# Zhen-Dong/CoDeNet

Measured on NVIDIA B200. Metric: CoDeNet1x 512x512 W4A8 forward + ctdet decode throughput, higher is better.
Workload: dtype int8

## Files before the change

### codenet_b200/csrc/decode.cu

```cuda
#include "layers.cuh"

#define DEC_THREADS 1024
#define DEC_BINS 2048
#define DEC_MAXK 1024

__device__ __forceinline__ uint32_t f2key(float f) {
  uint32_t b = __float_as_uint(f);
  return (b & 0x80000000u) ? ~b : (b | 0x80000000u);
}
__device__ __forceinline__ float key2f(uint32_t k) {
  uint32_t b = (k & 0x80000000u) ? (k & 0x7fffffffu) : ~k;
  return __uint_as_float(b);
}

struct DecParams {
  const float* hm; const float* wh; const float* reg;
  long long hm_is, wh_is, reg_is;
  int cat, H, W, K;
  int is_prob;
  unsigned long long* list;
  unsigned int* counts;
  float* dets; int32_t* inds;
};

__global__ void __launch_bounds__(256) ctdet_peaks_kernel(DecParams p, int batch) {
  const int HW = p.H * p.W;
  const unsigned n = (unsigned)p.cat * HW;
  const unsigned e = blockIdx.x * 256u + threadIdx.x;
  const int b = blockIdx.y, lane = threadIdx.x & 31;
  bool peak = false; float v = 0.f;
  if (e < n) {
    const int sp = (int)(e % (unsigned)HW); const int y = sp / p.W, x = sp - y * p.W;
    const float* plane = p.hm + (size_t)b * p.hm_is + (e - sp);
    v = __ldg(plane + sp);
    peak = (v == v);
#pragma unroll
    for (int dy = -1; dy <= 1; ++dy) {
      const int yy = y + dy; if ((unsigned)yy >= (unsigned)p.H) continue;
#pragma unroll
      for (int dx = -1; dx <= 1; ++dx) {
        const int xx = x + dx; if ((dx | dy) == 0 || (unsigned)xx >= (unsigned)p.W) continue;
        if (__ldg(plane + yy * p.W + xx) > v) peak = false;
      }
    }
  }
  __shared__ unsigned s_wcnt[8], s_base;
  const unsigned m = __ballot_sync(0xffffffffu, peak);
  const int warp = threadIdx.x >> 5;
  if (lane == 0) s_wcnt[warp] = __popc(m);
  __syncthreads();
  if (threadIdx.x == 0) {
    unsigned tot = 0;
#pragma unroll
    for (int w = 0; w < 8; ++w) { const unsigned c = s_wcnt[w]; s_wcnt[w] = tot; tot += c; }
    s_base = tot ? atomicAdd(p.counts + b, tot) : 0u;
  }
  __syncthreads();
  if (peak) p.list[(size_t)b * n + s_base + s_wcnt[warp] + __popc(m & ((1u << lane) - 1u))] =
      ((unsigned long long)f2key(v) << 32) | (unsigned long long)(0xffffffffu - e);
}

#define DEC_STRIP 16
__global__ void __launch_bounds__(256) ctdet_peaks_rows_kernel(DecParams p, int strips_per_plane) {
  pdl_launch_dependents();
  const int HW = p.H * p.W, W4 = p.W >> 2;
  const unsigned n = (unsigned)p.cat * HW;
  const int b = blockIdx.y, lane = threadIdx.x & 31, warp = threadIdx.x >> 5;
  const unsigned tid = blockIdx.x * 256u + threadIdx.x;
  const unsigned per_plane = (unsigned)strips_per_plane * W4;
  const unsigned plane_i = tid / per_plane, rem = tid - plane_i * per_plane;
  const bool live = plane_i < (unsigned)p.cat;
  const int strip = (int)(rem / W4), x0 = (int)(rem % W4) * 4;
  const float* plane = p.hm + (size_t)b * p.hm_is + (size_t)(live ? plane_i : 0) * HW;
  const int y0 = strip * DEC_STRIP, y1 = min(y0 + DEC_STRIP, p.H);
  const float NEG = -3.402823466e38f;
  auto load_row = [&](int y, float (&v)[4], float (&hm3)[4]) {
    if ((unsigned)y >= (unsigned)p.H || !live) { v[0] = v[1] = v[2] = v[3] = NEG; hm3[0] = hm3[1] = hm3[2] = hm3[3] = NEG; return; }
    const float* r = plane + (size_t)y * p.W + x0;
    const float4 q = __ldg((const float4*)r);
    const float l = x0 > 0 ? __ldg(r - 1) : NEG, rr = x0 + 4 < p.W ? __ldg(r + 4) : NEG;
    v[0] = q.x; v[1] = q.y; v[2] = q.z; v[3] = q.w;
    hm3[0] = fmaxf(fmaxf(l, q.x), q.y); hm3[1] = fmaxf(fmaxf(q.x, q.y), q.z);
    hm3[2] = fmaxf(fmaxf(q.y, q.z), q.w); hm3[3] = fmaxf(fmaxf(q.z, q.w), rr);
  };
  float vm[4], hmm[4], vc[4], hmc[4], vp[4], hmp[4];
  load_row(y0 - 1, vm, hmm); load_row(y0, vc, hmc);
  __shared__ unsigned s_wcnt[8], s_base;
  unsigned long long mask = 0ull;
  for (int y = y0; y < y1; ++y) {
    load_row(y + 1, vp, hmp);
#pragma unroll
    for (int i = 0; i < 4; ++i) {
      const float m = fmaxf(fmaxf(hmm[i], hmc[i]), hmp[i]);
      if (live && vc[i] == m) mask |= 1ull << ((y - y0) * 4 + i);
    }
#pragma unroll
    for (int i = 0; i < 4; ++i) { vm[i] = vc[i]; hmm[i] = hmc[i]; vc[i] = vp[i]; hmc[i] = hmp[i]; }
  }
  const unsigned cnt = (unsigned)__popcll(mask);
  unsigned incl = cnt;
#pragma unroll
  for (int o = 1; o < 32; o <<= 1) { const unsigned t = __shfl_up_sync(0xffffffffu, incl, o); if (lane >= o) incl += t; }
  if (lane == 31) s_wcnt[warp] = incl;
  __syncthreads();
  if (threadIdx.x == 0) {
    unsigned tot = 0;
#pragma unroll
    for (int w = 0; w < 8; ++w) { const unsigned c = s_wcnt[w]; s_wcnt[w] = tot; tot += c; }
    s_base = tot ? atomicAdd(p.counts + b, tot) : 0u;
  }
  __syncthreads();
  unsigned long long* dst = p.list + (size_t)b * n + s_base + s_wcnt[warp] + (incl - cnt);
  while (mask) {
    const int bit = __ffsll((long long)mask) - 1;
    mask &= mask - 1;
    const int y = y0 + (bit >> 2), x = x0 + (bit & 3);
    const float v = __ldg(plane + (size_t)y * p.W + x);
    const unsigned e = plane_i * HW + (unsigned)y * p.W + x;
    *dst++ = ((unsigned long long)f2key(v) << 32) | (unsigned long long)(0xffffffffu - e);
  }
}

__global__ void __launch_bounds__(DEC_THREADS) ctdet_decode_kernel(DecParams p) {
  __shared__ unsigned int hist[DEC_BINS];
  __shared__ unsigned long long sel[DEC_MAXK];
  __shared__ unsigned int s_count, s_nsel;
  __shared__ unsigned long long s_prefix, s_mask;
  __shared__ unsigned int s_krem, s_done;
  __shared__ unsigned int warp_sums[32];

  const int b = blockIdx.x, tid = threadIdx.x, lane = tid & 31, warp = tid >> 5;
  const int HW = p.H * p.W;
  const long long n = (long long)p.cat * HW;
  const float* hm = p.hm + (size_t)b * p.hm_is;
  unsigned long long* list = p.list + (size_t)b * n;

  if (tid == 0) { s_count = p.counts[b]; s_nsel = 0; }
  __syncthreads();
  const unsigned int count = s_count;
  const unsigned int Ksel = min((unsigned)p.K, count);

  if (tid == 0) { s_prefix = 0ull; s_mask = 0ull; s_krem = Ksel; s_done = (Ksel == 0 || Ksel == count) ? 1u : 0u; }
  __syncthreads();
  for (int shift = 53; !s_done; shift = max(shift - 11, 0)) {
    const int width = (shift == 0) ? 9 : 11;
    const unsigned nb = 1u << width;
    for (int i = tid; i < DEC_BINS; i += DEC_THREADS) hist[i] = 0;
    __syncthreads();
    const unsigned long long prefix = s_prefix, mask = s_mask;
    for (unsigned i = tid; i < count; i += DEC_THREADS) {
      unsigned long long c = list[i];
      if ((c & mask) == prefix) atomicAdd(&hist[(unsigned)(c >> shift) & (nb - 1)], 1u);
    }
    __syncthreads();
    {
      unsigned d0 = nb - 1 - 2 * tid, d1 = nb - 2 - 2 * tid;
      unsigned c0 = (2 * tid < nb) ? hist[d0] : 0u, c1 = (2 * tid + 1 < nb) ? hist[d1] : 0u;
      unsigned mine = c0 + c1, incl = mine;
      for (int o = 1; o < 32; o <<= 1) { unsigned t = __shfl_up_sync(0xffffffffu, incl, o); if (lane >= o) incl += t; }
      if (lane == 31) warp_sums[warp] = incl;
      __syncthreads();
      unsigned woff = 0;
      for (int w2 = 0; w2 < warp; ++w2) woff += warp_sums[w2];
      unsigned before = woff + incl - mine;
      const unsigned krem = s_krem;
      __syncthreads();
      if (2 * tid < nb && before < krem && krem <= before + c0) {
        s_prefix = prefix | ((unsigned long long)d0 << shift);
        s_mask = mask | ((unsigned long long)(nb - 1) << shift);
        s_krem = krem - before;
        if (krem == before + c0 || shift == 0) s_done = 1u;
      } else if (2 * tid + 1 < nb && before + c0 < krem && krem <= before + c0 + c1) {
        s_prefix = prefix | ((unsigned long long)d1 << shift);
        s_mask = mask | ((unsigned long long)(nb - 1) << shift);
        s_krem = krem - before - c0;
        if (krem == before + c0 + c1 || shift == 0) s_done = 1u;
      }
      __syncthreads();
    }
    if (shift == 0) break;
  }
  __syncthreads();
  const unsigned long long thr = (Ksel == count) ? 0ull : s_prefix;
  for (unsigned i = tid; i < count && Ksel > 0; i += DEC_THREADS) {
    unsigned long long c = list[i];
    if (c >= thr) { unsigned pos = atomicAdd(&s_nsel, 1u); if (pos < DEC_MAXK) sel[pos] = c; }
  }
  __syncthreads();
  unsigned nsel = min(s_nsel, (unsigned)DEC_MAXK);
  unsigned np2 = 1; while (np2 < nsel) np2 <<= 1;
  for (unsigned i = nsel + tid; i < np2; i += DEC_THREADS) sel[i] = 0ull;
  __syncthreads();
  for (unsigned k2 = 2; k2 <= np2; k2 <<= 1)
    for (unsigned j = k2 >> 1; j > 0; j >>= 1) {
      for (unsigned i = tid; i < np2; i += DEC_THREADS) {
        unsigned ixj = i ^ j;
        if (ixj > i) {
          unsigned long long a = sel[i], c = sel[ixj];
          bool desc = ((i & k2) == 0);
          if (desc ? (a < c) : (a > c)) { sel[i] = c; sel[ixj] = a; }
        }
      }
      __syncthreads();
    }
  for (int i = tid; i < p.K; i += DEC_THREADS) {
    float* d = p.dets + ((size_t)b * p.K + i) * 6;
    if ((unsigned)i < nsel && (unsigned)i < Ksel) {
      unsigned long long c = sel[i];
      uint32_t flat = 0xffffffffu - (uint32_t)(c & 0xffffffffull);
      float logit = key2f((uint32_t)(c >> 32));
      int cls = flat / HW, sp = flat - cls * HW;
      float xs = (float)(sp % p.W), ys = (float)(sp / p.W);
      if (p.reg) { xs += p.reg[(size_t)b * p.reg_is + sp]; ys += p.reg[(size_t)b * p.reg_is + HW + sp]; }
      else { xs += 0.5f; ys += 0.5f; }
      float w = p.wh[(size_t)b * p.wh_is + sp], h = p.wh[(size_t)b * p.wh_is + HW + sp];
      d[0] = xs - w / 2; d[1] = ys - h / 2; d[2] = xs + w / 2; d[3] = ys + h / 2;
      d[4] = p.is_prob ? logit : (float)(1.0 / (1.0 + exp(-(double)logit)));
      d[5] = (float)cls;
      if (p.inds) p.inds[(size_t)b * p.K + i] = (int32_t)flat;
    } else {
      d[0] = d[1] = d[2] = d[3] = d[4] = d[5] = 0.f;
      if (p.inds) p.inds[(size_t)b * p.K + i] = -1;
    }
  }
}

int decode_launch(const float* hm, long long hm_img_stride, const float* wh, long long wh_img_stride, const float* reg,
                  long long reg_img_stride, int batch, int cat, int H, int W, int K, int is_prob,
                  unsigned long long* scratch, unsigned int* counts, float* dets, int32_t* inds, cudaStream_t st) {
  CDN_CHECK(K >= 1 && K <= DEC_MAXK, CDN_ERR_INVALID, "decode: K=%d must be in 1..%d", K, DEC_MAXK);
  CDN_CHECK(cat >= 1 && H >= 1 && W >= 1 && (long long)cat * H * W < (1ll << 31), CDN_ERR_INVALID, "decode: bad shape");
  CDN_CHECK(hm && wh && dets && scratch && counts, CDN_ERR_INVALID, "decode: null pointer");
  CDN_CHECK(batch <= 65535, CDN_ERR_INVALID, "decode: batch %d exceeds 65535", batch);
  if (batch == 0) return 0;
  DecParams p{hm, wh, reg, hm_img_stride, wh_img_stride, reg_img_stride, cat, H, W, K, is_prob, scratch, counts, dets, inds};
  CDN_CUDA(cudaMemsetAsync(counts, 0, (size_t)batch * sizeof(unsigned int), st));
  const unsigned n = (unsigned)cat * H * W;
  if (W % 4 == 0 && (((uintptr_t)hm | (uintptr_t)(hm_img_stride * 4)) & 15) == 0) {
    const int strips = (H + DEC_STRIP - 1) / DEC_STRIP;
    const unsigned threads = (unsigned)cat * strips * (W / 4);
    ctdet_peaks_rows_kernel<<<dim3((threads + 255) / 256, batch), 256, 0, st>>>(p, strips);
    CDN_LAUNCH_CHECK("ctdet_peaks_rows_kernel");
  } else {
    ctdet_peaks_kernel<<<dim3((n + 255) / 256, batch), 256, 0, st>>>(p, batch);
    CDN_LAUNCH_CHECK("ctdet_peaks_kernel");
  }
  ctdet_decode_kernel<<<batch, DEC_THREADS, 0, st>>>(p);
  CDN_LAUNCH_CHECK("ctdet_decode_kernel");
  return 0;
}

__global__ void ctdet_post_affine_kernel(float* dets, const double* trans, int K, long long total) {
  const long long i = (long long)blockIdx.x * blockDim.x + threadIdx.x;
  if (i >= total) return;
  const double* t = trans + (i / K) * 6;
  float* d = dets + i * 6;
#pragma unroll
  for (int c = 0; c < 2; ++c) {
    const double x = (double)d[2 * c], y = (double)d[2 * c + 1];
    const double nx = __dadd_rn(__dadd_rn(__dmul_rn(t[0], x), __dmul_rn(t[1], y)), t[2]);
    const double ny = __dadd_rn(__dadd_rn(__dmul_rn(t[3], x), __dmul_rn(t[4], y)), t[5]);
    d[2 * c] = (float)nx; d[2 * c + 1] = (float)ny;
  }
}

extern "C" int cdn_ctdet_post_affine(float* d_dets, int batch, int K, const double* h_trans, cdn_stream_t stream) {
  CDN_CHECK(d_dets && h_trans && batch >= 0 && K >= 1, CDN_ERR_INVALID, "post_affine: bad arguments");
  if (batch == 0) return 0;
  double* d_t = nullptr;
  CDN_CUDA(cudaMalloc(&d_t, (size_t)batch * 6 * sizeof(double)));
// ... 40 lines not shown
```

### codenet_b200/csrc/engine.cu

```cuda
#include "layers.cuh"
#include <algorithm>
#include <mutex>

static thread_local char g_err[1024] = "";
unsigned g_cdn_debug_flags = 0;

int cdn_fail(int code, const char* fmt, ...) {
  va_list ap; va_start(ap, fmt); vsnprintf(g_err, sizeof(g_err), fmt, ap); va_end(ap);
  return code;
}
std::mutex& cdn_attr_mutex() { static std::mutex m; return m; }
int cdn_num_sms() {
  static int sms[64] = {};
  int dev = 0;
  if (cudaGetDevice(&dev) != cudaSuccess || dev < 0 || dev >= 64) return 148;
  std::lock_guard<std::mutex> lk(cdn_attr_mutex());
  if (!sms[dev]) { cudaDeviceGetAttribute(&sms[dev], cudaDevAttrMultiProcessorCount, dev); if (sms[dev] <= 0) sms[dev] = 148; }
  return sms[dev];
}

int dev_requant_upload(DevRequant& d, const cdn_requant* rq, const int32_t* acc_bias_host, int n_pad) {
  CDN_CHECK(rq && rq->n <= n_pad, CDN_ERR_INVALID, "requant: n=%d exceeds padded size %d", rq ? rq->n : -1, n_pad);
  std::vector<float> Mh(n_pad, 0.f), Bh(n_pad, 0.f), thr(n_pad, 0.5f);
  std::vector<double> M(n_pad, 0.0), B(n_pad, 0.0);
// ... 225 lines not shown
  if (int r = dw_device_build(L->dw, wq, sc->ws, C, pitch, zx, rq)) { delete L; return r; }
  if (int r = deform_scale_build(L->dw, &L->sc, L->ws.data(), C, zx)) { dw_device_free(L->dw); delete L; return r; }
  *out = L;
  return 0;
}
extern "C" int cdn_deform_layer_run(cdn_deform_layer* L, const int8_t* d_in, int in_pitch, int batch, int H, int W, int in_shift,
                                    int8_t* d_out, int out_pitch, float* d_sval, cdn_stream_t stream) {
  CDN_CHECK(L != nullptr, CDN_ERR_INVALID, "null deform layer");
  CDN_CHECK(std::min(in_pitch, out_pitch) >= L->Cp, CDN_ERR_INVALID, "deform layer: pitch smaller than the layer's %d", L->Cp);
  return deform_launch(L->dw, &L->sc, d_in, in_pitch, d_out, out_pitch, batch, H, W, in_shift, L->zx, d_sval, (cudaStream_t)stream);
}
extern "C" int cdn_deform_layer_destroy(cdn_deform_layer* L) {
  if (!L) return 0;
  cudaSetDevice(L->device);
  dw_device_free(L->dw);
  delete L;
  return 0;
}

static int decode_standalone(const float* d_hm, const float* d_wh, const float* d_reg, int batch, int cat, int H, int W,
                             int K, int is_prob, float* d_dets, int32_t* d_inds, cdn_stream_t stream) {
  unsigned long long* scratch = nullptr;
  CDN_CHECK(batch >= 0 && cat >= 1 && H >= 1 && W >= 1, CDN_ERR_INVALID, "decode: bad shape");
  size_t n = (size_t)batch * cat * H * W;
  CDN_CUDA(cudaMalloc(&scratch, (n ? n : 1) * sizeof(unsigned long long) + ((size_t)batch + 1) * sizeof(unsigned int)));
  long long hw = (long long)H * W;
  int r = decode_launch(d_hm, cat * hw, d_wh, 2 * hw, d_reg, 2 * hw, batch, cat, H, W, K, is_prob, scratch,
                        (unsigned int*)(scratch + (n ? n : 1)), d_dets, d_inds, (cudaStream_t)stream);
  cudaError_t e = cudaStreamSynchronize((cudaStream_t)stream);
  if (!r && e != cudaSuccess) r = cdn_fail(CDN_ERR_CUDA, "decode: %s", cudaGetErrorString(e));
  cudaFree(scratch);
  return r;
}
extern "C" size_t cdn_ctdet_decode_ws_bytes(int batch, int cat, int H, int W) {
  if (batch < 0 || cat < 1 || H < 1 || W < 1) return 0;
  size_t n = (size_t)batch * cat * H * W;
  return (n ? n : 1) * sizeof(unsigned long long) + ((size_t)batch + 1) * sizeof(unsigned int);
}
extern "C" int cdn_ctdet_decode_ws(const float* d_hm, long long hm_img_stride, const float* d_wh, long long wh_img_stride,
                                   const float* d_reg, long long reg_img_stride, int batch, int cat, int H, int W,
                                   int K, int is_prob, float* d_dets, int32_t* d_inds, void* d_ws, size_t ws_bytes,
                                   cdn_stream_t stream) {
  CDN_CHECK(batch >= 0 && cat >= 1 && H >= 1 && W >= 1, CDN_ERR_INVALID, "decode: bad shape");
  CDN_CHECK(d_ws && ((uintptr_t)d_ws & 7) == 0 && ws_bytes >= cdn_ctdet_decode_ws_bytes(batch, cat, H, W), CDN_ERR_INVALID,
            "decode: workspace of %zu bytes (8-byte aligned) needed, got %zu", cdn_ctdet_decode_ws_bytes(batch, cat, H, W), ws_bytes);
  size_t n = (size_t)batch * cat * H * W;
  long long hw = (long long)H * W;
  CDN_CHECK((!hm_img_stride || hm_img_stride >= cat * hw) && (!wh_img_stride || wh_img_stride >= 2 * hw) &&
            (!reg_img_stride || reg_img_stride >= 2 * hw), CDN_ERR_INVALID, "decode: image stride smaller than one image");
  unsigned long long* scratch = (unsigned long long*)d_ws;
  return decode_launch(d_hm, hm_img_stride ? hm_img_stride : cat * hw, d_wh, wh_img_stride ? wh_img_stride : 2 * hw, d_reg,
                       reg_img_stride ? reg_img_stride : 2 * hw, batch, cat, H, W, K, is_prob, scratch,
                       (unsigned int*)(scratch + (n ? n : 1)), d_dets, d_inds, (cudaStream_t)stream);
}
extern "C" int cdn_ctdet_decode(const float* d_hm, const float* d_wh, const float* d_reg, int batch, int cat, int H, int W,
                                int K, float* d_dets, int32_t* d_inds, cdn_stream_t stream) {
  return decode_standalone(d_hm, d_wh, d_reg, batch, cat, H, W, K, 0, d_dets, d_inds, stream);
}
extern "C" int cdn_ctdet_decode_prob(const float* d_heat, const float* d_wh, const float* d_reg, int batch, int cat, int H,
                                     int W, int K, float* d_dets, int32_t* d_inds, cdn_stream_t stream) {
  return decode_standalone(d_heat, d_wh, d_reg, batch, cat, H, W, K, 1, d_dets, d_inds, stream);
}

struct EngTensor { int H, W, pitch; int8_t* ptr; };
struct EngOp {
  int kind;
  int in_t, pass_t, out_t, in_shift, stride, pool, zx, H, W;
  StemDevice stem; DwDevice dw; PwDevice pw; cdn_deform_scale sc; std::vector<int8_t> ws_host;
  CUtensorMap tmA, tmP, tmO;
};

struct cdn_engine {
  int device = 0, max_batch = 0, finalized = 0;
  int in_H = 0, in_W = 0;
  std::vector<EngTensor> tensors;
  std::vector<EngOp*> ops;
// ... 162 lines not shown
}

extern "C" int cdn_engine_set_heads(cdn_engine* e, int cat, int H, int W, int K, int has_reg) {
  ENG_CHECK(e);
  CDN_CHECK(cat > 0 && H > 0 && W > 0 && K > 0 && K <= 1024, CDN_ERR_INVALID, "heads: bad arguments");
  e->cat = cat; e->hH = H; e->hW = W; e->K = K; e->has_reg = has_reg;
  return 0;
}

extern "C" int cdn_engine_finalize(cdn_engine* e, int max_batch) {
  ENG_CHECK(e);
  CDN_CHECK(!e->finalized, CDN_ERR_STATE, "engine already finalized");
  CDN_CHECK(max_batch > 0 && !e->ops.empty() && e->cat > 0, CDN_ERR_INVALID, "finalize: empty plan, heads not set, or bad batch");
  CDN_CHECK(e->n_f32 == e->cat + 2 + (e->has_reg ? 2 : 0), CDN_ERR_INVALID, "finalize: head conv has %d fp32 planes, expected %d", e->n_f32, e->cat + 2 + (e->has_reg ? 2 : 0));
  CDN_CUDA(cudaSetDevice(e->device));
  e->max_batch = max_batch;
  for (auto& t : e->tensors) {
    size_t bytes = (size_t)max_batch * t.H * t.W * t.pitch;
    CDN_CUDA(cudaMalloc((void**)&t.ptr, bytes));
    CDN_CUDA(cudaMemset(t.ptr, 0, bytes));
  }
  size_t ppi = (size_t)e->hH * e->hW;
  CDN_CUDA(cudaMalloc((void**)&e->heads, (size_t)max_batch * e->n_f32 * ppi * sizeof(float)));
  CDN_CUDA(cudaMalloc((void**)&e->dec_scratch, (size_t)max_batch * e->cat * ppi * sizeof(unsigned long long) + ((size_t)max_batch + 1) * sizeof(unsigned int)));
  CDN_CUDA(cudaMalloc((void**)&e->dets, (size_t)max_batch * e->K * 6 * sizeof(float)));
  CDN_CUDA(cudaMalloc((void**)&e->inds, (size_t)max_batch * e->K * sizeof(int32_t)));
  for (auto* op : e->ops) {
    if (op->kind == 0 && op->pool) {
      size_t b = (size_t)max_batch * ((op->H - 1) / op->stride + 1) * ((op->W - 1) / op->stride + 1) * 32;
      CDN_CUDA(cudaMalloc((void**)&e->stem_tmp, b));
    }
    if (op->kind == 3) {
      const EngTensor& ti = e->tensors[op->in_t];
      uint64_t rows = (uint64_t)max_batch * ti.H * ti.W;
      if (int r = make_tmap_2d(&op->tmA, ti.ptr, ti.pitch, rows, ti.pitch, 128)) return r;
      if (op->pass_t >= 0) { const EngTensor& tp = e->tensors[op->pass_t]; if (int r = make_tmap_2d(&op->tmP, tp.ptr, tp.pitch, rows, tp.pitch, 128)) return r; }
      if (op->out_t >= 0) { const EngTensor& to = e->tensors[op->out_t]; if (int r = make_tmap_2d(&op->tmO, to.ptr, to.pitch, rows, to.pitch, 128)) return r; }
    }
  }
  CDN_CUDA(cudaDeviceSynchronize());
  e->finalized = 1;
  return 0;
}

static bool engine_fuses_heads(const cdn_engine* e, size_t oi) {
  if (!e->fuse_heads || (g_cdn_debug_flags & 256u) || oi + 1 >= e->ops.size()) return false;
  const EngOp *a = e->ops[oi], *b = e->ops[oi + 1];
// ... 95 lines not shown
        int out_pitch = op->out_t >= 0 ? e->tensors[op->out_t].pitch : 0;
        r = pw_launch(op->pw, ti.ptr, ti.pitch, (long long)batch * ti.H * ti.W, pass, pass_pitch, out, out_pitch,
                      op->out_t < 0 ? e->heads : nullptr, e->hH * e->hW, &op->tmA, op->pass_t >= 0 ? &op->tmP : nullptr,
                      op->out_t >= 0 ? &op->tmO : nullptr, st);
        launches++;
      } break;
    }
    if (r) return r;
    mark();
  }
  const long long ppi = (long long)e->hH * e->hW;
  if (d_hm || d_wh || d_reg) {
    long long total = (long long)batch * e->n_f32 * ppi;
    heads_copyout_kernel<<<(unsigned)((total + 255) / 256), 256, 0, st>>>(e->heads, e->n_f32, e->cat, (int)ppi, total, d_hm, d_wh, d_reg, e->hm_logits);
    CDN_LAUNCH_CHECK("heads_copyout_kernel");
    launches++;
  }
  mark();
  if (d_dets) {
    const float* hm = e->heads;
    const float* wh = e->heads + (size_t)e->cat * ppi;
    const float* reg = e->has_reg ? e->heads + (size_t)(e->cat + 2) * ppi : nullptr;
    long long is = (long long)e->n_f32 * ppi;
    if (int r = decode_launch(hm, is, wh, is, reg, is, batch, e->cat, e->hH, e->hW, e->K, 0, e->dec_scratch,
                              (unsigned int*)(e->dec_scratch + (size_t)e->max_batch * e->cat * ppi), d_dets, d_inds, st)) return r;
    launches += 2;
  }
  mark();
  e->launches = launches;
  return 0;
}

extern "C" int cdn_engine_profile(cdn_engine* e, const float* d_img, int batch, float* ms, int n, cdn_stream_t stream) {
  ENG_CHECK(e);
  CDN_CHECK(e->finalized && batch > 0 && batch <= e->max_batch && d_img && ms, CDN_ERR_INVALID, "profile: bad arguments");
  CDN_CHECK(n >= (int)e->ops.size() + 2, CDN_ERR_INVALID, "profile: need room for %d timings", (int)e->ops.size() + 2);
  CDN_CUDA(cudaSetDevice(e->device));
  std::vector<cudaEvent_t> marks;
  int r = engine_enqueue(e, d_img, 0, batch, nullptr, nullptr, nullptr, e->dets, e->inds, (cudaStream_t)stream, &marks);
  cudaError_t ce = cudaStreamSynchronize((cudaStream_t)stream);
  if (!r && ce != cudaSuccess) r = cdn_fail(CDN_ERR_CUDA, "profile: %s", cudaGetErrorString(ce));
  for (int i = 0; i < n; ++i) ms[i] = 0.f;
  if (!r) for (size_t i = 0; i + 1 < marks.size() && (int)i < n; ++i) cudaEventElapsedTime(&ms[i], marks[i], marks[i + 1]);
  for (auto ev : marks) cudaEventDestroy(ev);
  return r;
}

static int engine_run_any(cdn_engine* e, const void* d_img, int is_u8, int batch, float* d_hm, float* d_wh, float* d_reg,
// ... 200 lines not shown
```

### codenet_b200/csrc/layers.cuh

```cuda
#pragma once
#include "common.cuh"

struct DwDevice {
  uint32_t *wA = nullptr, *wB = nullptr, *wC = nullptr, *ws = nullptr;
  uint32_t *wpk1 = nullptr, *wpk2 = nullptr, *wpku = nullptr;
  float2* mb = nullptr; int32_t* abm = nullptr; float thr = 0.5f, thr_bil = 0.01f; int u_ok = 1;
  RqInt* ki = nullptr; int use_int = 0;
  int sh0 = 0;
  uint32_t* pad_px = nullptr;
  int32_t* s_thr = nullptr; int s_n = 0, s_lo = 0, s_mode0_ok = 0;
  DevRequant rq;
  int cw_total = 0;
  long long acc_s_bias = 0;
};
int dw_device_build(DwDevice& d, const int8_t* wq, const int8_t* ws, int C, int Cp, int zx, const cdn_requant* rq);
int deform_scale_build(DwDevice& d, const cdn_deform_scale* sc, const int8_t* ws, int C, int zx);
void dw_device_free(DwDevice& d);
int dw_launch(const DwDevice& d, const int8_t* in, int in_pitch, int8_t* out, int out_pitch, int batch, int H, int W,
              int in_shift, int stride, int zx, cudaStream_t st);
bool dw_tma_ok(const DwDevice& d, int in_pitch, int out_pitch, int H, int W, int in_shift, int stride);
int dw_tma_launch(const DwDevice& d, const int8_t* in, int in_pitch, int8_t* out, int out_pitch, int batch, int H, int W,
                  int stride, int zx, cudaStream_t st);
int deform_launch(const DwDevice& d, const cdn_deform_scale* sc, const int8_t* in, int in_pitch, int8_t* out,
                  int out_pitch, int batch, int H, int W, int in_shift, int zx, float* sval, cudaStream_t st);
// ... 36 lines not shown
int pw_launch(const PwDevice& d, const int8_t* in, int in_pitch, long long pixels, const int8_t* pass, int pass_pitch,
              int8_t* out, int out_pitch, float* out_f32, int ppi, const CUtensorMap* tmA, const CUtensorMap* tmP,
              const CUtensorMap* tmO, cudaStream_t st);
bool heads_fused_ok(const DwDevice& dw, const PwDevice& pw, int in_pitch, int mid_pitch, int Hs, int Ws);
int heads_fused_launch(const DwDevice& dw, const PwDevice& pw, const int8_t* in, int in_pitch, int batch, int Hs, int Ws,
                       int zx, float* out_f32, cudaStream_t st);
bool unit_fused_ok(const PwDevice& pw1, const DwDevice& dw, const PwDevice& pw3, int x_pitch, int mid_pitch, int out_pitch, int H, int W);
int unit_fused_launch(const PwDevice& pw1, const DwDevice& dw, const PwDevice& pw3, const int8_t* x, int8_t* out, int HP,
                      int batch, int H, int W, int zx_mid, int8_t* dump_c1, int8_t* dump_d2, cudaStream_t st);
bool unit_fused_ws_ok(const PwDevice& pw1, const DwDevice& dw, const PwDevice& pw3, int x_pitch, int mid_pitch, int out_pitch, int H, int W);
int unit_fused_ws_launch(const PwDevice& pw1, const DwDevice& dw, const PwDevice& pw3, const int8_t* x, int8_t* out,
                         int batch, int H, int W, int zx_mid, int8_t* dump_c1, int8_t* dump_d2, cudaStream_t st);
int make_tmap_nhwc_swz(CUtensorMap* m, const void* base, uint64_t pitch, uint64_t W, uint64_t H, uint64_t batch,
                       uint32_t box_c, uint32_t box_w, uint32_t box_h);
bool unit_s2_fused_ok(const PwDevice& pw1, const DwDevice& dw, const PwDevice& pw3, int x_pitch, int mid_pitch, int pass_pitch,
                      int out_pitch, int H, int W);
int unit_s2_fused_launch(const PwDevice& pw1, const DwDevice& dw, const PwDevice& pw3, const int8_t* x, const int8_t* pass, int pass_pitch,
                         int8_t* out, int batch, int H, int W, int zx_mid, int8_t* dump_c1, int8_t* dump_d2, cudaStream_t st);
int make_tmap_nhwc(CUtensorMap* m, const void* base, uint64_t pitch, uint64_t W, uint64_t H, uint64_t batch, uint32_t box_w, uint32_t box_h);
int make_tmap_2d(CUtensorMap* m, const void* base, uint64_t cols, uint64_t rows, uint64_t pitch, uint32_t box_rows);

int decode_launch(const float* hm, long long hm_img_stride, const float* wh, long long wh_img_stride, const float* reg,
                  long long reg_img_stride, int batch, int cat, int H, int W, int K, int is_prob,
                  unsigned long long* scratch, unsigned int* counts, float* dets, int32_t* inds, cudaStream_t st);
```

Measured before the change: 93520.

## Replace global peak list with per-block local top-K slots before final selection

Each peak-finding block now keeps a shared histogram of its local peaks and runs a radix top-K select, writing at most K candidates into a fixed per-block slot region. The old design appended every peak to one global list through an atomic counter. The final decode kernel then runs radix select over the much smaller slot array, staging it in dynamic shared memory when it fits, and the counts memset is removed. This cuts global traffic and the cost of the single-block selection, but adds per-block selection work and zero-padded slots.

New measurement: 93270, median of 6. No clear change (-0.3%).

```diff
diff --git a/codenet_b200/csrc/decode.cu b/codenet_b200/csrc/decode.cu
--- a/codenet_b200/csrc/decode.cu
+++ b/codenet_b200/csrc/decode.cu
@@ -1,8 +1,17 @@
 #include "layers.cuh"
 
+#include <algorithm>
+
+#ifndef DEC_THREADS
 #define DEC_THREADS 1024
+#endif
+#define DEC_RT 256
+#define DEC_STRIP 16
+#define DEC_EPT 16
 #define DEC_BINS 2048
 #define DEC_MAXK 1024
+#define DEC_STAGE 2048
+#define DEC_SMEM_CAND 12288
 
 __device__ __forceinline__ uint32_t f2key(float f) {
   uint32_t b = __float_as_uint(f);
@@ -11,6 +20,9 @@
 __device__ __forceinline__ float key2f(uint32_t k) {
   uint32_t b = (k & 0x80000000u) ? (k & 0x7fffffffu) : ~k;
   return __uint_as_float(b);
+}
+__device__ __forceinline__ unsigned long long composite(float v, unsigned e) {
+  return ((unsigned long long)f2key(v) << 32) | (unsigned long long)(0xffffffffu - e);
 }
 
 struct DecParams {
@@ -18,22 +30,114 @@
   long long hm_is, wh_is, reg_is;
   int cat, H, W, K;
   int is_prob;
-  unsigned long long* list;
-  unsigned int* counts;
+  int rpp, spr, kslot;
+  unsigned nslots;
+  unsigned long long* slots;
   float* dets; int32_t* inds;
 };
 
-__global__ void __launch_bounds__(256) ctdet_peaks_kernel(DecParams p, int batch) {
+struct DecSel { unsigned warp[32]; unsigned res[4]; unsigned pos, nst; };
+
+template <int NT>
+__device__ void radix_find(const unsigned* hist, unsigned nb, unsigned krem, DecSel& s) {
+  const unsigned t = threadIdx.x, lane = t & 31, warp = t >> 5;
+  const unsigned per = (nb + NT - 1) / NT, r0 = t * per;
+  unsigned mine = 0;
+  for (unsigned j = 0; j < per && r0 + j < nb; ++j) mine += hist[nb - 1 - r0 - j];
+  unsigned incl = mine;
+#pragma unroll
+  for (int o = 1; o < 32; o <<= 1) { const unsigned v = __shfl_up_sync(0xffffffffu, incl, o); if (lane >= (unsigned)o) incl += v; }
+  if (lane == 31) s.warp[warp] = incl;
+  __syncthreads();
+  unsigned before = incl - mine, total = 0;
+#pragma unroll
+  for (unsigned w = 0; w < NT / 32; ++w) { const unsigned c = s.warp[w]; total += c; if (w < warp) before += c; }
+  if (before < krem && krem <= before + mine) {
+    for (unsigned j = 0;; ++j) {
+      const unsigned d = nb - 1 - r0 - j, c = hist[d];
+      if (krem <= before + c) { s.res[0] = d; s.res[1] = before; s.res[2] = c; break; }
+      before += c;
+    }
+  }
+  if (t == 0) s.res[3] = total;
+  __syncthreads();
+}
+
+template <int NT, class Each>
+__device__ unsigned long long topk_threshold(Each&& each, unsigned* hist, unsigned kk, DecSel& s, unsigned& total) {
+  __syncthreads();
+  unsigned nb = DEC_BINS, krem = kk;
+  int shift = 53;
+  radix_find<NT>(hist, nb, krem, s);
+  total = s.res[3];
+  if (total <= kk) return 0ull;
+  unsigned long long prefix = 0ull, pmask = 0ull;
+  for (;;) {
+    prefix |= (unsigned long long)s.res[0] << shift;
+    pmask |= (unsigned long long)(nb - 1) << shift;
+    krem -= s.res[1];
+    if (krem == s.res[2] || shift == 0) return prefix;
+    shift = max(shift - 11, 0);
+    nb = shift ? DEC_BINS : 512;
+    for (unsigned i = threadIdx.x; i < nb; i += NT) hist[i] = 0;
+    __syncthreads();
+    each([&](unsigned long long c) {
+      if ((c & pmask) == prefix) atomicAdd(&hist[(unsigned)(c >> shift) & (nb - 1)], 1u);
+    });
+    __syncthreads();
+    radix_find<NT>(hist, nb, krem, s);
+  }
+}
+
+template <class Each>
+__device__ void region_topk(Each&& each, unsigned* hist, DecSel& s, unsigned kslot, unsigned long long* out) {
+  __shared__ unsigned long long stage[DEC_STAGE];
+  if (threadIdx.x == 0) { s.pos = 0; s.nst = 0; }
+  __syncthreads();
+  radix_find<DEC_RT>(hist, DEC_BINS, kslot, s);
+  const unsigned total = s.res[3], d1 = s.res[0], c1 = s.res[2];
+  if (total <= kslot) {
+    each([&](unsigned long long c) { out[atomicAdd(&s.pos, 1u)] = c; });
+    for (unsigned i = total + threadIdx.x; i < kslot; i += DEC_RT) out[i] = 0ull;
+    return;
+  }
+  if (c1 <= DEC_STAGE) {
+    const unsigned krem = kslot - s.res[1];
+    each([&](unsigned long long c) {
+      const unsigned d = (unsigned)(c >> 53);
+      if (d > d1) out[atomicAdd(&s.pos, 1u)] = c;
+      else if (d == d1) stage[atomicAdd(&s.nst, 1u)] = c;
+    });
+    for (unsigned i = threadIdx.x; i < DEC_BINS; i += DEC_RT) hist[i] = 0;
+    __syncthreads();
+    if (threadIdx.x == 0) hist[d1] = c1;
+    auto each_staged = [&](auto&& f) { for (unsigned i = threadIdx.x; i < c1; i += DEC_RT) f(stage[i]); };
+    unsigned t;
+    const unsigned long long thr = topk_threshold<DEC_RT>(each_staged, hist, krem, s, t);
+    each_staged([&](unsigned long long c) { if (c >= thr) out[atomicAdd(&s.pos, 1u)] = c; });
+    return;
+  }
+  unsigned t;
+  const unsigned long long thr = topk_threshold<DEC_RT>(each, hist, kslot, s, t);
+  each([&](unsigned long long c) { if (c >= thr) out[atomicAdd(&s.pos, 1u)] = c; });
+}
+
+__global__ void __launch_bounds__(DEC_RT) ctdet_peaks_kernel(DecParams p) {
+  __shared__ unsigned s_hist[DEC_BINS];
+  __shared__ DecSel s;
+  for (unsigned i = threadIdx.x; i < DEC_BINS; i += DEC_RT) s_hist[i] = 0;
   const int HW = p.H * p.W;
-  const unsigned n = (unsigned)p.cat * HW;
-  const unsigned e = blockIdx.x * 256u + threadIdx.x;
-  const int b = blockIdx.y, lane = threadIdx.x & 31;
-  bool peak = false; float v = 0.f;
-  if (e < n) {
-    const int sp = (int)(e % (unsigned)HW); const int y = sp / p.W, x = sp - y * p.W;
-    const float* plane = p.hm + (size_t)b * p.hm_is + (e - sp);
-    v = __ldg(plane + sp);
-    peak = (v == v);
+  const int b = blockIdx.y, plane_i = blockIdx.x / p.rpp, sp0 = (blockIdx.x - plane_i * p.rpp) * (DEC_RT * DEC_EPT);
+  const float* plane = p.hm + (size_t)b * p.hm_is + (size_t)plane_i * HW;
+  __syncthreads();
+  unsigned mask = 0;
+#pragma unroll 4
+  for (int j = 0; j < DEC_EPT; ++j) {
+    const int sp = sp0 + j * DEC_RT + threadIdx.x;
+    if (sp >= HW) break;
+    const int y = sp / p.W, x = sp - y * p.W;
+    const float v = __ldg(plane + sp);
+    bool peak = (v == v) && (v >= -3.402823466e38f || (y > 0 && y < p.H - 1 && x > 0 && x < p.W - 1));
 #pragma unroll
     for (int dy = -1; dy <= 1; ++dy) {
       const int yy = y + dy; if ((unsigned)yy >= (unsigned)p.H) continue;
@@ -43,153 +147,116 @@
         if (__ldg(plane + yy * p.W + xx) > v) peak = false;
       }
     }
-  }
-  __shared__ unsigned s_wcnt[8], s_base;
-  const unsigned m = __ballot_sync(0xffffffffu, peak);
-  const int warp = threadIdx.x >> 5;
-  if (lane == 0) s_wcnt[warp] = __popc(m);
-  __syncthreads();
-  if (threadIdx.x == 0) {
-    unsigned tot = 0;
-#pragma unroll
-    for (int w = 0; w < 8; ++w) { const unsigned c = s_wcnt[w]; s_wcnt[w] = tot; tot += c; }
-    s_base = tot ? atomicAdd(p.counts + b, tot) : 0u;
-  }
-  __syncthreads();
-  if (peak) p.list[(size_t)b * n + s_base + s_wcnt[warp] + __popc(m & ((1u << lane) - 1u))] =
-      ((unsigned long long)f2key(v) << 32) | (unsigned long long)(0xffffffffu - e);
-}
-
-#define DEC_STRIP 16
-__global__ void __launch_bounds__(256) ctdet_peaks_rows_kernel(DecParams p, int strips_per_plane) {
+    if (peak) { mask |= 1u << j; atomicAdd(&s_hist[f2key(v) >> 21], 1u); }
+  }
+  const unsigned base = (unsigned)plane_i * HW;
+  region_topk([&](auto&& f) {
+    for (unsigned m = mask; m; m &= m - 1) {
+      const int sp = sp0 + (__ffs(m) - 1) * DEC_RT + threadIdx.x;
+      f(composite(__ldg(plane + sp), base + sp));
+    }
+  }, s_hist, s, p.kslot, p.slots + ((size_t)b * gridDim.x + blockIdx.x) * p.kslot);
+}
+
+__global__ void __launch_bounds__(DEC_RT) ctdet_peaks_rows_kernel(DecParams p) {
   pdl_launch_dependents();
+  __shared__ unsigned s_hist[DEC_BINS];
+  __shared__ DecSel s;
+  for (unsigned i = threadIdx.x; i < DEC_BINS; i += DEC_RT) s_hist[i] = 0;
   const int HW = p.H * p.W, W4 = p.W >> 2;
-  const unsigned n = (unsigned)p.cat * HW;
-  const int b = blockIdx.y, lane = threadIdx.x & 31, warp = threadIdx.x >> 5;
-  const unsigned tid = blockIdx.x * 256u + threadIdx.x;
-  const unsigned per_plane = (unsigned)strips_per_plane * W4;
-  const unsigned plane_i = tid / per_plane, rem = tid - plane_i * per_plane;
-  const bool live = plane_i < (unsigned)p.cat;
-  const int strip = (int)(rem / W4), x0 = (int)(rem % W4) * 4;
-  const float* plane = p.hm + (size_t)b * p.hm_is + (size_t)(live ? plane_i : 0) * HW;
-  const int y0 = strip * DEC_STRIP, y1 = min(y0 + DEC_STRIP, p.H);
+  const int b = blockIdx.y, plane_i = blockIdx.x / p.rpp, r = blockIdx.x - plane_i * p.rpp;
+  const int ls = threadIdx.x / W4, x0 = (threadIdx.x - ls * W4) * 4;
+  const int y0 = (r * p.spr + ls) * DEC_STRIP, y1 = min(y0 + DEC_STRIP, p.H);
+  const float* plane = p.hm + (size_t)b * p.hm_is + (size_t)plane_i * HW;
   const float NEG = -3.402823466e38f;
-  auto load_row = [&](int y, float (&v)[4], float (&hm3)[4]) {
-    if ((unsigned)y >= (unsigned)p.H || !live) { v[0] = v[1] = v[2] = v[3] = NEG; hm3[0] = hm3[1] = hm3[2] = hm3[3] = NEG; return; }
-    const float* r = plane + (size_t)y * p.W + x0;
-    const float4 q = __ldg((const float4*)r);
-    const float l = x0 > 0 ? __ldg(r - 1) : NEG, rr = x0 + 4 < p.W ? __ldg(r + 4) : NEG;
-    v[0] = q.x; v[1] = q.y; v[2] = q.z; v[3] = q.w;
-    hm3[0] = fmaxf(fmaxf(l, q.x), q.y); hm3[1] = fmaxf(fmaxf(q.x, q.y), q.z);
-    hm3[2] = fmaxf(fmaxf(q.y, q.z), q.w); hm3[3] = fmaxf(fmaxf(q.z, q.w), rr);
+  struct Row { float4 q; float l, r; };
+  auto load_row = [&](int y) {
+    Row o;
+    if ((unsigned)y < (unsigned)p.H) {
+      const float* rp = plane + (size_t)y * p.W + x0;
+      o.q = __ldg((const float4*)rp);
+      o.l = x0 > 0 ? __ldg(rp - 1) : NEG; o.r = x0 + 4 < p.W ? __ldg(rp + 4) : NEG;
+    } else {
+      o.q = make_float4(NEG, NEG, NEG, NEG); o.l = o.r = NEG;
+    }
+    return o;
   };
-  float vm[4], hmm[4], vc[4], hmc[4], vp[4], hmp[4];
-  load_row(y0 - 1, vm, hmm); load_row(y0, vc, hmc);
-  __shared__ unsigned s_wcnt[8], s_base;
+  auto hmax3 = [](const Row& o, float (&h)[4]) {
+    h[0] = fmaxf(fmaxf(o.l, o.q.x), o.q.y); h[1] = fmaxf(fmaxf(o.q.x, o.q.y), o.q.z);
+    h[2] = fmaxf(fmaxf(o.q.y, o.q.z), o.q.w); h[3] = fmaxf(fmaxf(o.q.z, o.q.w), o.r);
+  };
+  __syncthreads();
   unsigned long long mask = 0ull;
-  for (int y = y0; y < y1; ++y) {
-    load_row(y + 1, vp, hmp);
-#pragma unroll
-    for (int i = 0; i < 4; ++i) {
-      const float m = fmaxf(fmaxf(hmm[i], hmc[i]), hmp[i]);
-      if (live && vc[i] == m) mask |= 1ull << ((y - y0) * 4 + i);
-    }
-#pragma unroll
-    for (int i = 0; i < 4; ++i) { vm[i] = vc[i]; hmm[i] = hmc[i]; vc[i] = vp[i]; hmc[i] = hmp[i]; }
-  }
-  const unsigned cnt = (unsigned)__popcll(mask);
-  unsigned incl = cnt;
-#pragma unroll
-  for (int o = 1; o < 32; o <<= 1) { const unsigned t = __shfl_up_sync(0xffffffffu, incl, o); if (lane >= o) incl += t; }
-  if (lane == 31) s_wcnt[warp] = incl;
-  __syncthreads();
-  if (threadIdx.x == 0) {
-    unsigned tot = 0;
-#pragma unroll
-    for (int w = 0; w < 8; ++w) { const unsigned c = s_wcnt[w]; s_wcnt[w] = tot; tot += c; }
-    s_base = tot ? atomicAdd(p.counts + b, tot) : 0u;
-  }
-  __syncthreads();
-  unsigned long long* dst = p.list + (size_t)b * n + s_base + s_wcnt[warp] + (incl - cnt);
-  while (mask) {
-    const int bit = __ffsll((long long)mask) - 1;
-    mask &= mask - 1;
-    const int y = y0 + (bit >> 2), x = x0 + (bit & 3);
-    const float v = __ldg(plane + (size_t)y * p.W + x);
-    const unsigned e = plane_i * HW + (unsigned)y * p.W + x;
-    *dst++ = ((unsigned long long)f2key(v) << 32) | (unsigned long long)(0xffffffffu - e);
-  }
-}
-
-__global__ void __launch_bounds__(DEC_THREADS) ctdet_decode_kernel(DecParams p) {
+  if (ls < p.spr && y0 < p.H) {
+    Row rm = load_row(y0 - 1), rc = load_row(y0), rp = load_row(y0 + 1);
+#pragma unroll 1
+    for (int k = 0; k < DEC_STRIP; ++k) {
+      const int y = y0 + k;
+      if (y >= y1) break;
+      const Row rn = load_row(y + 2 <= y1 ? y + 2 : -1);
+      float hm[4], hc[4], hp[4];
+      hmax3(rm, hm); hmax3(rc, hc); hmax3(rp, hp);
+      const float v[4] = {rc.q.x, rc.q.y, rc.q.z, rc.q.w};
+#pragma unroll
+      for (int i = 0; i < 4; ++i) {
+        if (v[i] == fmaxf(fmaxf(hm[i], hc[i]), hp[i])) {
+          mask |= 1ull << (k * 4 + i);
+          atomicAdd(&s_hist[f2key(v[i]) >> 21], 1u);
+        }
+      }
+      rm = rc; rc = rp; rp = rn;
+    }
+  }
+  const unsigned base = (unsigned)plane_i * HW;
+  region_topk([&](auto&& f) {
+#pragma unroll 1
+    for (int k0 = 0; k0 < DEC_STRIP; k0 += 2) {
+      const unsigned m8 = (unsigned)(mask >> (k0 * 4)) & 0xffu;
+      if (!m8) continue;
+      float4 q[2];
+#pragma unroll
+      for (int k = 0; k < 2; ++k)
+        if (m8 >> (k * 4) & 15u) q[k] = __ldg((const float4*)(plane + (size_t)(y0 + k0 + k) * p.W + x0));
+#pragma unroll
+      for (int k = 0; k < 2; ++k) {
+        const unsigned e = (unsigned)(y0 + k0 + k) * p.W + x0;
+        const float v[4] = {q[k].x, q[k].y, q[k].z, q[k].w};
+#pragma unroll
+        for (int i = 0; i < 4; ++i) if (m8 >> (k * 4 + i) & 1u) f(composite(v[i], base + e + i));
+      }
+    }
+  }, s_hist, s, p.kslot, p.slots + ((size_t)b * gridDim.x + blockIdx.x) * p.kslot);
+}
+
+__global__ void __launch_bounds__(DEC_THREADS) ctdet_decode_kernel(DecParams p, int in_smem) {
+  extern __shared__ unsigned long long s_cand[];
   __shared__ unsigned int hist[DEC_BINS];
   __shared__ unsigned long long sel[DEC_MAXK];
-  __shared__ unsigned int s_count, s_nsel;
-  __shared__ unsigned long long s_prefix, s_mask;
-  __shared__ unsigned int s_krem, s_done;
-  __shared__ unsigned int warp_sums[32];
-
-  const int b = blockIdx.x, tid = threadIdx.x, lane = tid & 31, warp = tid >> 5;
+  __shared__ DecSel s;
+
+  const int b = blockIdx.x, tid = threadIdx.x;
   const int HW = p.H * p.W;
-  const long long n = (long long)p.cat * HW;
-  const float* hm = p.hm + (size_t)b * p.hm_is;
-  unsigned long long* list = p.list + (size_t)b * n;
-
-  if (tid == 0) { s_count = p.counts[b]; s_nsel = 0; }
-  __syncthreads();
-  const unsigned int count = s_count;
-  const unsigned int Ksel = min((unsigned)p.K, count);
-
-  if (tid == 0) { s_prefix = 0ull; s_mask = 0ull; s_krem = Ksel; s_done = (Ksel == 0 || Ksel == count) ? 1u : 0u; }
-  __syncthreads();
-  for (int shift = 53; !s_done; shift = max(shift - 11, 0)) {
-    const int width = (shift == 0) ? 9 : 11;
-    const unsigned nb = 1u << width;
-    for (int i = tid; i < DEC_BINS; i += DEC_THREADS) hist[i] = 0;
-    __syncthreads();
-    const unsigned long long prefix = s_prefix, mask = s_mask;
-    for (unsigned i = tid; i < count; i += DEC_THREADS) {
-      unsigned long long c = list[i];
-      if ((c & mask) == prefix) atomicAdd(&hist[(unsigned)(c >> shift) & (nb - 1)], 1u);
-    }
-    __syncthreads();
-    {
-      unsigned d0 = nb - 1 - 2 * tid, d1 = nb - 2 - 2 * tid;
-      unsigned c0 = (2 * tid < nb) ? hist[d0] : 0u, c1 = (2 * tid + 1 < nb) ? hist[d1] : 0u;
-      unsigned mine = c0 + c1, incl = mine;
-      for (int o = 1; o < 32; o <<= 1) { unsigned t = __shfl_up_sync(0xffffffffu, incl, o); if (lane >= o) incl += t; }
-      if (lane == 31) warp_sums[warp] = incl;
-      __syncthreads();
-      unsigned woff = 0;
-      for (int w2 = 0; w2 < warp; ++w2) woff += warp_sums[w2];
-      unsigned before = woff + incl - mine;
-      const unsigned krem = s_krem;
-      __syncthreads();
-      if (2 * tid < nb && before < krem && krem <= before + c0) {
-        s_prefix = prefix | ((unsigned long long)d0 << shift);
-        s_mask = mask | ((unsigned long long)(nb - 1) << shift);
-        s_krem = krem - before;
-        if (krem == before + c0 || shift == 0) s_done = 1u;
-      } else if (2 * tid + 1 < nb && before + c0 < krem && krem <= before + c0 + c1) {
-        s_prefix = prefix | ((unsigned long long)d1 << shift);
-        s_mask = mask | ((unsigned long long)(nb - 1) << shift);
-        s_krem = krem - before - c0;
-        if (krem == before + c0 + c1 || shift == 0) s_done = 1u;
-      }
-      __syncthreads();
-    }
-    if (shift == 0) break;
-  }
-  __syncthreads();
-  const unsigned long long thr = (Ksel == count) ? 0ull : s_prefix;
-  for (unsigned i = tid; i < count && Ksel > 0; i += DEC_THREADS) {
-    unsigned long long c = list[i];
-    if (c >= thr) { unsigned pos = atomicAdd(&s_nsel, 1u); if (pos < DEC_MAXK) sel[pos] = c; }
-  }
-  __syncthreads();
-  unsigned nsel = min(s_nsel, (unsigned)DEC_MAXK);
-  unsigned np2 = 1; while (np2 < nsel) np2 <<= 1;
-  for (unsigned i = nsel + tid; i < np2; i += DEC_THREADS) sel[i] = 0ull;
+  const unsigned n = p.nslots;
+  const unsigned long long* g = p.slots + (size_t)b * n;
+  for (int i = tid; i < DEC_BINS; i += DEC_THREADS) hist[i] = 0;
+  if (tid == 0) s.pos = 0;
+  __syncthreads();
+  for (unsigned i = tid; i < n; i += DEC_THREADS) {
+    const unsigned long long c = g[i];
+    if (in_smem) s_cand[i] = c;
+    if (c) atomicAdd(&hist[(unsigned)(c >> 53)], 1u);
+  }
+  const unsigned long long* cand = in_smem ? s_cand : g;
+  auto each = [&](auto&& f) {
+    for (unsigned i = tid; i < n; i += DEC_THREADS) { const unsigned long long c = cand[i]; if (c) f(c); }
+  };
+  unsigned count;
+  const unsigned long long thr = topk_threshold<DEC_THREADS>(each, hist, (unsigned)p.K, s, count);
+  const unsigned Ksel = min((unsigned)p.K, count);
+  each([&](unsigned long long c) { if (c >= thr) sel[atomicAdd(&s.pos, 1u)] = c; });
+  __syncthreads();
+  unsigned np2 = 1; while (np2 < Ksel) np2 <<= 1;
+  for (unsigned i = Ksel + tid; i < np2; i += DEC_THREADS) sel[i] = 0ull;
   __syncthreads();
   for (unsigned k2 = 2; k2 <= np2; k2 <<= 1)
     for (unsigned j = k2 >> 1; j > 0; j >>= 1) {
@@ -205,7 +272,7 @@
     }
   for (int i = tid; i < p.K; i += DEC_THREADS) {
     float* d = p.dets + ((size_t)b * p.K + i) * 6;
-    if ((unsigned)i < nsel && (unsigned)i < Ksel) {
+    if ((unsigned)i < Ksel) {
       unsigned long long c = sel[i];
       uint32_t flat = 0xffffffffu - (uint32_t)(c & 0xffffffffull);
       float logit = key2f((uint32_t)(c >> 32));
@@ -225,27 +292,59 @@
   }
 }
 
+struct DecGeom { int rows, rpp, spr, kslot; long long slots; };
+static DecGeom dec_geom(int cat, int H, int W, int K, bool rows) {
+  DecGeom g{rows ? 1 : 0, 0, 0, 0, 0};
+  long long region;
+  if (rows) {
+    const int strips = (H + DEC_STRIP - 1) / DEC_STRIP;
+    g.spr = DEC_RT / (W / 4);
+    g.rpp = (strips + g.spr - 1) / g.spr;
+    region = (long long)std::min(g.spr * DEC_STRIP, H) * W;
+  } else {
+    const long long HW = (long long)H * W;
+    g.rpp = (int)((HW + DEC_RT * DEC_EPT - 1) / (DEC_RT * DEC_EPT));
+    region = std::min<long long>(HW, DEC_RT * DEC_EPT);
+  }
+  g.kslot = (int)std::min<long long>(K, region);
+  g.slots = (long long)cat * g.rpp * g.kslot;
+  return g;
+}
+static bool dec_rows_ok(const float* hm, long long hm_img_stride, int W) {
+  return W % 4 == 0 && W / 4 <= DEC_RT && (((uintptr_t)hm | (uintptr_t)(hm_img_stride * 4)) & 15) == 0;
+}
+
+size_t decode_scratch_bytes(int batch, int cat, int H, int W, int K) {
+  long long slots = dec_geom(cat, H, W, K, false).slots;
+  if (W % 4 == 0 && W / 4 <= DEC_RT) slots = std::max(slots, dec_geom(cat, H, W, K, true).slots);
+  return std::max<size_t>((size_t)batch * slots, 1) * sizeof(unsigned long long);
+}
+
 int decode_launch(const float* hm, long long hm_img_stride, const float* wh, long long wh_img_stride, const float* reg,
                   long long reg_img_stride, int batch, int cat, int H, int W, int K, int is_prob,
-                  unsigned long long* scratch, unsigned int* counts, float* dets, int32_t* inds, cudaStream_t st) {
+                  unsigned long long* scratch, float* dets, int32_t* inds, cudaStream_t st) {
   CDN_CHECK(K >= 1 && K <= DEC_MAXK, CDN_ERR_INVALID, "decode: K=%d must be in 1..%d", K, DEC_MAXK);
   CDN_CHECK(cat >= 1 && H >= 1 && W >= 1 && (long long)cat * H * W < (1ll << 31), CDN_ERR_INVALID, "decode: bad shape");
-  CDN_CHECK(hm && wh && dets && scratch && counts, CDN_ERR_INVALID, "decode: null pointer");
+  CDN_CHECK(hm && wh && dets && scratch, CDN_ERR_INVALID, "decode: null pointer");
   CDN_CHECK(batch <= 65535, CDN_ERR_INVALID, "decode: batch %d exceeds 65535", batch);
   if (batch == 0) return 0;
-  DecParams p{hm, wh, reg, hm_img_stride, wh_img_stride, reg_img_stride, cat, H, W, K, is_prob, scratch, counts, dets, inds};
-  CDN_CUDA(cudaMemsetAsync(counts, 0, (size_t)batch * sizeof(unsigned int), st));
-  const unsigned n = (unsigned)cat * H * W;
-  if (W % 4 == 0 && (((uintptr_t)hm | (uintptr_t)(hm_img_stride * 4)) & 15) == 0) {
-    const int strips = (H + DEC_STRIP - 1) / DEC_STRIP;
-    const unsigned threads = (unsigned)cat * strips * (W / 4);
-    ctdet_peaks_rows_kernel<<<dim3((threads + 255) / 256, batch), 256, 0, st>>>(p, strips);
+  const DecGeom g = dec_geom(cat, H, W, K, dec_rows_ok(hm, hm_img_stride, W));
+  CDN_CHECK(g.slots <= (long long)cat * H * W, CDN_ERR_INVALID, "decode: %lld slots exceed the map", g.slots);
+  DecParams p{hm, wh, reg, hm_img_stride, wh_img_stride, reg_img_stride, cat, H, W, K, is_prob,
+              g.rpp, g.spr, g.kslot, (unsigned)g.slots, scratch, dets, inds};
+  const dim3 grid((unsigned)(cat * g.rpp), batch);
+  if (g.rows) {
+    ctdet_peaks_rows_kernel<<<grid, DEC_RT, 0, st>>>(p);
     CDN_LAUNCH_CHECK("ctdet_peaks_rows_kernel");
   } else {
-    ctdet_peaks_kernel<<<dim3((n + 255) / 256, batch), 256, 0, st>>>(p, batch);
+    ctdet_peaks_kernel<<<grid, DEC_RT, 0, st>>>(p);
     CDN_LAUNCH_CHECK("ctdet_peaks_kernel");
   }
-  ctdet_decode_kernel<<<batch, DEC_THREADS, 0, st>>>(p);
+  static bool attr_set[64];
+  if (cdn_first_on_device(attr_set))
+    CDN_CUDA(cudaFuncSetAttribute(ctdet_decode_kernel, cudaFuncAttributeMaxDynamicSharedMemorySize, DEC_SMEM_CAND * 8));
+  const int in_smem = g.slots <= DEC_SMEM_CAND;
+  ctdet_decode_kernel<<<batch, DEC_THREADS, in_smem ? (size_t)g.slots * 8 : 0, st>>>(p, in_smem);
   CDN_LAUNCH_CHECK("ctdet_decode_kernel");
   return 0;
 }
diff --git a/codenet_b200/csrc/engine.cu b/codenet_b200/csrc/engine.cu
--- a/codenet_b200/csrc/engine.cu
+++ b/codenet_b200/csrc/engine.cu
@@ -271,11 +271,10 @@
                              int K, int is_prob, float* d_dets, int32_t* d_inds, cdn_stream_t stream) {
   unsigned long long* scratch = nullptr;
   CDN_CHECK(batch >= 0 && cat >= 1 && H >= 1 && W >= 1, CDN_ERR_INVALID, "decode: bad shape");
-  size_t n = (size_t)batch * cat * H * W;
-  CDN_CUDA(cudaMalloc(&scratch, (n ? n : 1) * sizeof(unsigned long long) + ((size_t)batch + 1) * sizeof(unsigned int)));
+  CDN_CUDA(cudaMalloc(&scratch, decode_scratch_bytes(batch, cat, H, W, K)));
   long long hw = (long long)H * W;
-  int r = decode_launch(d_hm, cat * hw, d_wh, 2 * hw, d_reg, 2 * hw, batch, cat, H, W, K, is_prob, scratch,
-                        (unsigned int*)(scratch + (n ? n : 1)), d_dets, d_inds, (cudaStream_t)stream);
+  int r = decode_launch(d_hm, cat * hw, d_wh, 2 * hw, d_reg, 2 * hw, batch, cat, H, W, K, is_prob, scratch, d_dets, d_inds,
+                        (cudaStream_t)stream);
   cudaError_t e = cudaStreamSynchronize((cudaStream_t)stream);
   if (!r && e != cudaSuccess) r = cdn_fail(CDN_ERR_CUDA, "decode: %s", cudaGetErrorString(e));
   cudaFree(scratch);
@@ -293,14 +292,12 @@
   CDN_CHECK(batch >= 0 && cat >= 1 && H >= 1 && W >= 1, CDN_ERR_INVALID, "decode: bad shape");
   CDN_CHECK(d_ws && ((uintptr_t)d_ws & 7) == 0 && ws_bytes >= cdn_ctdet_decode_ws_bytes(batch, cat, H, W), CDN_ERR_INVALID,
             "decode: workspace of %zu bytes (8-byte aligned) needed, got %zu", cdn_ctdet_decode_ws_bytes(batch, cat, H, W), ws_bytes);
-  size_t n = (size_t)batch * cat * H * W;
   long long hw = (long long)H * W;
   CDN_CHECK((!hm_img_stride || hm_img_stride >= cat * hw) && (!wh_img_stride || wh_img_stride >= 2 * hw) &&
             (!reg_img_stride || reg_img_stride >= 2 * hw), CDN_ERR_INVALID, "decode: image stride smaller than one image");
-  unsigned long long* scratch = (unsigned long long*)d_ws;
   return decode_launch(d_hm, hm_img_stride ? hm_img_stride : cat * hw, d_wh, wh_img_stride ? wh_img_stride : 2 * hw, d_reg,
-                       reg_img_stride ? reg_img_stride : 2 * hw, batch, cat, H, W, K, is_prob, scratch,
-                       (unsigned int*)(scratch + (n ? n : 1)), d_dets, d_inds, (cudaStream_t)stream);
+                       reg_img_stride ? reg_img_stride : 2 * hw, batch, cat, H, W, K, is_prob, (unsigned long long*)d_ws,
+                       d_dets, d_inds, (cudaStream_t)stream);
 }
 extern "C" int cdn_ctdet_decode(const float* d_hm, const float* d_wh, const float* d_reg, int batch, int cat, int H, int W,
                                 int K, float* d_dets, int32_t* d_inds, cdn_stream_t stream) {
@@ -509,7 +506,7 @@
   }
   size_t ppi = (size_t)e->hH * e->hW;
   CDN_CUDA(cudaMalloc((void**)&e->heads, (size_t)max_batch * e->n_f32 * ppi * sizeof(float)));
-  CDN_CUDA(cudaMalloc((void**)&e->dec_scratch, (size_t)max_batch * e->cat * ppi * sizeof(unsigned long long) + ((size_t)max_batch + 1) * sizeof(unsigned int)));
+  CDN_CUDA(cudaMalloc((void**)&e->dec_scratch, decode_scratch_bytes(max_batch, e->cat, e->hH, e->hW, e->K)));
   CDN_CUDA(cudaMalloc((void**)&e->dets, (size_t)max_batch * e->K * 6 * sizeof(float)));
   CDN_CUDA(cudaMalloc((void**)&e->inds, (size_t)max_batch * e->K * sizeof(int32_t)));
   for (auto* op : e->ops) {
@@ -651,8 +648,8 @@
     const float* wh = e->heads + (size_t)e->cat * ppi;
     const float* reg = e->has_reg ? e->heads + (size_t)(e->cat + 2) * ppi : nullptr;
     long long is = (long long)e->n_f32 * ppi;
-    if (int r = decode_launch(hm, is, wh, is, reg, is, batch, e->cat, e->hH, e->hW, e->K, 0, e->dec_scratch,
-                              (unsigned int*)(e->dec_scratch + (size_t)e->max_batch * e->cat * ppi), d_dets, d_inds, st)) return r;
+    if (int r = decode_launch(hm, is, wh, is, reg, is, batch, e->cat, e->hH, e->hW, e->K, 0, e->dec_scratch, d_dets, d_inds, st))
+      return r;
     launches += 2;
   }
   mark();
diff --git a/codenet_b200/csrc/layers.cuh b/codenet_b200/csrc/layers.cuh
--- a/codenet_b200/csrc/layers.cuh
+++ b/codenet_b200/csrc/layers.cuh
@@ -82,4 +82,5 @@
 
 int decode_launch(const float* hm, long long hm_img_stride, const float* wh, long long wh_img_stride, const float* reg,
                   long long reg_img_stride, int batch, int cat, int H, int W, int K, int is_prob,
-                  unsigned long long* scratch, unsigned int* counts, float* dets, int32_t* inds, cudaStream_t st);
+                  unsigned long long* scratch, float* dets, int32_t* inds, cudaStream_t st);
+size_t decode_scratch_bytes(int batch, int cat, int H, int W, int K);
```
